# LabJunBMI/E3-invaraint-diffusion-model

Hardware: AMD Instinct MI355X
Metric: denoising-steps/sec (batched pocket graphs) (higher is better)
Workload: dtype f32 storage and accumulation, f16x3 products (fp32 grade); 1 GPU; structure_model sampling step, 256 x 256-residue pockets per GPU, 12+12 layers x 768, T=1000 schedule, encoder recomputed every step (as the reference); pockets_per_gpu=256, seq_len=256, parallelism=pocket-sharded x1, no collective

## Files before the change

e3-invaraint-diffusion-model_amd/csrc/attn_relkey_coop.hip:

```cpp
#include <type_traits>

#include "e3d_common.h"

namespace {

typedef __bf16 bf16x8 __attribute__((ext_vector_type(8)));
typedef __bf16 bf16x4 __attribute__((ext_vector_type(4)));
typedef _Float16 f16x8 __attribute__((ext_vector_type(8)));
typedef _Float16 f16x4 __attribute__((ext_vector_type(4)));
template <typename E> struct AV;
template <> struct AV<__bf16> { typedef bf16x8 x8; typedef bf16x4 x4; };
template <> struct AV<_Float16> { typedef f16x8 x8; typedef f16x4 x4; };
template <typename X> struct Elem;
template <> struct Elem<bf16x8> { typedef __bf16 type; };
template <> struct Elem<bf16x4> { typedef __bf16 type; };
template <> struct Elem<f16x8> { typedef _Float16 type; };
template <> struct Elem<f16x4> { typedef _Float16 type; };
__device__ __forceinline__ f32x16 mma16(const bf16x8 a, const bf16x8 b, const f32x16 c) {
    return __builtin_amdgcn_mfma_f32_32x32x16_bf16(a, b, c, 0, 0, 0);
}
__device__ __forceinline__ f32x16 mma16(const f16x8 a, const f16x8 b, const f32x16 c) {
    return __builtin_amdgcn_mfma_f32_32x32x16_f16(a, b, c, 0, 0, 0);
}

constexpr int D = 64;
constexpr int RING_LD = 34;
constexpr int RING_F = 64 * RING_LD;
constexpr int OUT_LD = 68;
constexpr int K_ROW_B = 144;
constexpr int V_ROW_B = 192;
constexpr int K_PLANE_B = 32 * K_ROW_B, V_PLANE_B = 32 * V_ROW_B;
constexpr float LOG2E = 1.4426950408889634f, LN2 = 0.6931471805599453f;
constexpr float Q_SCALE = 0.125f * LOG2E;
constexpr float MASK_BIAS = -10000.0f * LOG2E;
float g_rescale_tau = 8.0f;
constexpr int KV_BUF_B = 2 * K_PLANE_B + 2 * V_PLANE_B + 128;

template <typename X4>
__device__ __forceinline__ void split4x2(const f32x4 v, X4& hi, X4& lo) {
    typedef typename Elem<X4>::type E;
#pragma unroll
    for (int j = 0; j < 4; ++j) {
        const E p = (E)v[j];
        hi[j] = p;
        lo[j] = (E)(v[j] - (float)p);
    }
}

template <typename X8>
__device__ __forceinline__ void split8x2(const float (&x)[8], X8& hi, X8& lo) {
    typedef typename Elem<X8>::type E;
#pragma unroll
    for (int j = 0; j < 8; ++j) {
        const E p = (E)x[j];
        hi[j] = p;
        lo[j] = (E)(x[j] - (float)p);
    }
}

__device__ __forceinline__ void split4x2(const f32x4 v, f16x4& hi, f16x4& lo) {
    e3d_f16x2 h0, l0, h1, l1;
    e3d_split2_f16(v[0], v[1], h0, l0);
    e3d_split2_f16(v[2], v[3], h1, l1);
    hi = f16x4{h0[0], h0[1], h1[0], h1[1]};
    lo = f16x4{l0[0], l0[1], l1[0], l1[1]};
}
__device__ __forceinline__ void split8x2(const float (&x)[8], f16x8& hi, f16x8& lo) {
#pragma unroll
    for (int j = 0; j < 8; j += 2) {
        e3d_f16x2 h, l;
        e3d_split2_f16(x[j], x[j + 1], h, l);
        hi[j] = h[0]; hi[j + 1] = h[1];
        lo[j] = l[0]; lo[j + 1] = l[1];
    }
}

template <typename X8>
__device__ __forceinline__ f32x16 mfma3(const X8 (&a)[2], const X8 (&b)[2], f32x16 acc) {
    acc = mma16(a[0], b[1], acc);
    acc = mma16(a[1], b[0], acc);
    acc = mma16(a[0], b[0], acc);
    return acc;
}

typedef short short4v __attribute__((ext_vector_type(4)));
typedef short short8v __attribute__((ext_vector_type(8)));
template <typename X8>
__device__ __forceinline__ X8 tr_read8(const unsigned char* lo4, const unsigned char* hi4) {
    typedef __attribute__((address_space(3))) short4v* lds_p;
    const short4v a = __builtin_amdgcn_ds_read_tr16_b64_v4i16((lds_p)(lo4));
    const short4v b = __builtin_amdgcn_ds_read_tr16_b64_v4i16((lds_p)(hi4));
    const short8v c = __builtin_shufflevector(a, b, 0, 1, 2, 3, 4, 5, 6, 7);
    return __builtin_bit_cast(X8, c);
}

template <typename E>
__global__ __launch_bounds__(256) void e_fragments_kernel(const float* __restrict__ e, typename AV<E>::x8* __restrict__ frag,
                                                          int P, int J0, int n_items, float* __restrict__ e_absmax) {
    const int i = blockIdx.x * 256 + threadIdx.x;
    if (i >= n_items) return;
    const int lane = i & 63, kb = (i >> 6) & 3, plane = (i >> 8) & 1, j = i >> 9;
    const int row = min(max(P + 32 * (j - J0) + (lane & 31), 0), 2 * P - 2);
    const float* src = e + row * D + 16 * kb + 8 * (lane >> 5);
    typename AV<E>::x8 out;
    unsigned amax = 0;
#pragma unroll
    for (int t = 0; t < 8; ++t) {
        const float v = src[t];
        const E hi = (E)v;
        out[t] = plane ? (E)(v - (float)hi) : hi;
        e3d_absmax_accum(amax, v);
    }
    frag[i] = out;
    if (e_absmax && plane == 0) e3d_absmax_commit(amax, e_absmax, lane);
}

#ifdef E3D_ATTN_STAMPS
__device__ long long e3d_attn_stamps[16][8];
#define ASTAMP(slot)                                                                                     \
    do {                                                                                                 \
        if (blockIdx.x == 1000 && wid == 1 && lane == 0 && kt < 16) e3d_attn_stamps[kt][slot] = __builtin_readcyclecounter(); \
    } while (0)
#define KSTAMP(i)                                                                                        \
    do {                                                                                                 \
        if (blockIdx.x == 1000 && wid == 1 && lane == 0) e3d_attn_stamps[15][i] = __builtin_readcyclecounter(); \
    } while (0)
#else
#define ASTAMP(slot) do {} while (0)
#define KSTAMP(i) do {} while (0)
#endif

template <int W, bool RELKEY, typename E, bool DROP = false>
__global__ __launch_bounds__(W * 64, 2) void attn_coop_kernel(
    const float* __restrict__ q, int64_t q_bs, int64_t q_rs, const float* __restrict__ k, int64_t k_bs,
    int64_t k_rs, const float* __restrict__ v, int64_t v_bs, int64_t v_rs, const typename AV<E>::x8* __restrict__ e_frag,
    int P, const float* __restrict__ key_mask, float* __restrict__ out, float* __restrict__ lse, int nh, int Lq, int Lk,
    int groups_per_bh, int skip_padded_tiles, E3dBounds bnd, float rescale_tau, E3dDrop drop_in) {
    const E3dDrop drop = e3d_drop_resolve(drop_in);
    typedef typename AV<E>::x8 bf16x8;
    typedef typename AV<E>::x4 bf16x4;
    extern __shared__ __attribute__((aligned(16))) unsigned char smem_raw[];
    constexpr int NT = W * 64, NI = 512 / NT;
    const int tid = threadIdx.x, lane = tid & 63, wid = tid >> 6;
    const int qi = lane & 31, half = lane >> 5;
    const int blk = xcd_remap(blockIdx.x, gridDim.x);
    const int grp = blk % groups_per_bh, bh = blk / groups_per_bh, h = bh % nh, b = bh / nh;
    const int q0 = (grp * W + wid) * 32;
    float* ring = reinterpret_cast<float*>(smem_raw + 2 * KV_BUF_B) + wid * RING_F;
    KSTAMP(0);

    const float* kb_ = k + b * k_bs + h * D;
    const float* vb_ = v + b * v_bs + h * D;
    const float* mb = key_mask ? key_mask + (int64_t)b * Lk : nullptr;
    f32x4 qraw[8];
    {
        const float* qrow = q + b * q_bs + (int64_t)min(q0 + qi, Lq - 1) * q_rs + h * D + 8 * half;
#pragma unroll
        for (int kb = 0; kb < 4; ++kb) {
            qraw[2 * kb] = *reinterpret_cast<const f32x4*>(qrow + 16 * kb);
            qraw[2 * kb + 1] = *reinterpret_cast<const f32x4*>(qrow + 16 * kb + 4);
        }
    }
    const bool scan_mask = mb && skip_padded_tiles && e3d_mask_skip_is_exact(bnd);
    float mv[4];
    {
        const float* mp = mb ? mb : kb_;
#pragma unroll
        for (int c = 0; c < 4; ++c) mv[c] = mp[min(64 * c + lane, Lk - 1)];
    }

    bf16x8 qf[4][2];
    int k_tiles = (Lk + 31) >> 5;

    constexpr bool DEEP = NI <= 2;
    constexpr int NSET = DEEP ? 2 : 1;
    f32x4 sk[NSET][NI], sv[NSET][NI];
    float smask[NSET];
    int voff_k[NI], voff_v[NI];
#pragma unroll
    for (int i = 0; i < NI; ++i) {
        const int f = tid + NT * i;
        voff_k[i] = ((f >> 4) * (int)k_rs + 4 * (f & 15)) * 4;
        voff_v[i] = ((f >> 4) * (int)v_rs + 4 * (f & 15)) * 4;
    }
    const int voff_m = (tid & 31) * 4;
    auto tile_rsrc = [&](const float* base, int64_t rs, int r0, int tail_floats) {
        const int rows = Lk - r0;
        return __builtin_amdgcn_make_buffer_rsrc(const_cast<float*>(base + (int64_t)r0 * rs), 0,
                                                 (int)(((int64_t)(rows - 1) * rs + tail_floats) * 4), 0x00020000);
    };
    auto stage_load = [&](auto set_tag, int r0) {
        constexpr int SET = decltype(set_tag)::value;
        const auto rk = tile_rsrc(kb_, k_rs, r0, D), rv = tile_rsrc(vb_, v_rs, r0, D);
#pragma unroll
        for (int i = 0; i < NI; ++i) {
            sk[SET][i] = __builtin_bit_cast(f32x4, __builtin_amdgcn_raw_buffer_load_b128(rk, voff_k[i], 0, 0));
            sv[SET][i] = __builtin_bit_cast(f32x4, __builtin_amdgcn_raw_buffer_load_b128(rv, voff_v[i], 0, 0));
        }
        const auto rm = tile_rsrc(mb ? mb : kb_, 1, r0, 1);
        const float mval = __builtin_bit_cast(float, __builtin_amdgcn_raw_buffer_load_b32(rm, voff_m, 0, 0));
        smask[SET] = mb ? mval : 1.0f;
    };
    auto stage_store = [&](auto set_tag, int r0, unsigned char* buf) {
        constexpr int SET = decltype(set_tag)::value;
#pragma unroll
        for (int i = 0; i < NI; ++i) {
            const int f = tid + NT * i, row = f >> 4, c4 = f & 15;
            bf16x4 hi, lo;
            split4x2(sk[SET][i], hi, lo);
            *reinterpret_cast<bf16x4*>(buf + row * K_ROW_B + 8 * c4) = hi;
            *reinterpret_cast<bf16x4*>(buf + K_PLANE_B + row * K_ROW_B + 8 * c4) = lo;
            split4x2(sv[SET][i], hi, lo);
            *reinterpret_cast<bf16x4*>(buf + 2 * K_PLANE_B + row * V_ROW_B + 8 * c4) = hi;
            *reinterpret_cast<bf16x4*>(buf + 2 * K_PLANE_B + V_PLANE_B + row * V_ROW_B + 8 * c4) = lo;
        }
        if (tid < 32)
            reinterpret_cast<float*>(buf + 2 * K_PLANE_B + 2 * V_PLANE_B)[tid] =
                r0 + tid < Lk ? (1.0f - smask[SET]) * MASK_BIAS : -INFINITY;
    };
    using Set0 = std::integral_constant<int, 0>;
    using Set1 = std::integral_constant<int, DEEP ? 1 : 0>;

    bf16x8 ef[4][2];
    const int J0 = (Lk + 31) >> 5, qt = q0 >> 5;
    const auto e_rsrc = __builtin_amdgcn_make_buffer_rsrc(const_cast<bf16x8*>(e_frag ? e_frag : reinterpret_cast<const bf16x8*>(k)), 0,
                                                          2 * ((Lk + 31) >> 5) * 512 * 16, 0x00020000);
    const int voff_e = lane * 16;
    auto e_load = [&](int j) {
        const int so = __builtin_amdgcn_readfirstlane(j * 8192);
#pragma unroll
        for (int kb = 0; kb < 4; ++kb) {
            ef[kb][0] = __builtin_bit_cast(bf16x8, __builtin_amdgcn_raw_buffer_load_b128(e_rsrc, voff_e + kb * 1024, so, 0));
            ef[kb][1] = __builtin_bit_cast(bf16x8, __builtin_amdgcn_raw_buffer_load_b128(e_rsrc, voff_e + kb * 1024, so + 4096, 0));
        }
    };
    auto dot_q_acc = [&](const bf16x8 (&x)[4][2], f32x16 acc) {
#pragma unroll
        for (int kb = 0; kb < 4; ++kb) acc = mfma3(x[kb], qf[kb], acc);
        return acc;
    };
    auto dot_q = [&](const bf16x8 (&x)[4][2]) {
        f32x16 acc;
#pragma unroll
        for (int r = 0; r < 16; ++r) acc[r] = 0.f;
        return dot_q_acc(x, acc);
    };

    stage_load(Set0{}, 0);
    if (RELKEY) e_load(qt + J0);

    if (scan_mask) {
        int last = -1;
#pragma unroll
        for (int c = 0; c < 4; ++c) {
            const bool valid = 64 * c + lane < Lk && mv[c] != 0.f;
            const unsigned long long bits = __ballot(valid);
            if (bits) last = 64 * c + 63 - __builtin_clzll(bits);
        }
        for (int base = 256; base < Lk; base += 64) {
            const int key = base + lane;
            const bool valid = key < Lk && mb[key] != 0.f;
            const unsigned long long bits = __ballot(valid);
            if (bits) last = base + 63 - __builtin_clzll(bits);
        }
        if (last >= 0) k_tiles = (last >> 5) + 1;
    }
#pragma unroll
    for (int kb = 0; kb < 4; ++kb) {
        const f32x4 lo4 = qraw[2 * kb], hi4 = qraw[2 * kb + 1];
        float x[8] = {lo4[0] * Q_SCALE, lo4[1] * Q_SCALE, lo4[2] * Q_SCALE, lo4[3] * Q_SCALE,
                      hi4[0] * Q_SCALE, hi4[1] * Q_SCALE, hi4[2] * Q_SCALE, hi4[3] * Q_SCALE};
#pragma unroll
        for (int j = 0; j < 8; ++j) asm volatile("" : "+v"(x[j]));
        split8x2(x, qf[kb][0], qf[kb][1]);
    }
    if (RELKEY) {
        f32x16 t = dot_q(ef);
        e_load(qt - 1 + J0);
#pragma unroll
        for (int r = 0; r < 16; ++r) ring[(32 + mfma32_row(r, half)) * RING_LD + qi] = t[r];
        t = dot_q(ef);
        e_load(qt - (k_tiles > 1 ? 1 : 0) - 1 + J0);
#pragma unroll
        for (int r = 0; r < 16; ++r) ring[mfma32_row(r, half) * RING_LD + qi] = t[r];
    }
    stage_store(Set0{}, 0, smem_raw);
    if (DEEP) stage_load(Set1{}, (k_tiles > 1 ? 1 : 0) * 32);
    __syncthreads();
    KSTAMP(1);

    f32x16 o0, o1;
#pragma unroll
    for (int r = 0; r < 16; ++r) { o0[r] = 0.f; o1[r] = 0.f; }
    float m_run = 0.f, l_run = 0.f;
    float* const ring_w = ring + 4 * half * RING_LD + qi;
    const float* const ring_e = ring + (qi + 31 - 4 * half - 27) * RING_LD + qi;
    int rd_odd[16];
    if (RELKEY) {
#pragma unroll
        for (int r = 0; r < 16; ++r) rd_odd[r] = (((qi - mfma32_row(r, half) + 31) ^ 32) * RING_LD + qi);
    }

    auto tile = [&](auto par_tag, int kt) {
        constexpr int PAR = decltype(par_tag)::value;
        const unsigned char* buf = smem_raw + PAR * KV_BUF_B;
        const bool more = kt + 1 < k_tiles;
        const int kt_next = more ? kt + 1 : kt;
        ASTAMP(0);
        ASTAMP(1);

        const float* kbias = reinterpret_cast<const float*>(buf + 2 * K_PLANE_B + 2 * V_PLANE_B);
        f32x16 s;
#pragma unroll
        for (int g = 0; g < 4; ++g) {
            const f32x4 bv = *reinterpret_cast<const f32x4*>(kbias + 8 * g + 4 * half);
#pragma unroll
            for (int j = 0; j < 4; ++j) s[4 * g + j] = bv[j] - m_run;
        }
        if (RELKEY) {
#pragma unroll
            for (int r = 0; r < 16; ++r)
                s[r] += PAR ? ring[rd_odd[r]] : ring_e[(27 - ((r & 3) + 8 * (r >> 2))) * RING_LD];
        }
        {
            bf16x8 kf[4][2];
            const unsigned char* kr = buf + qi * K_ROW_B + 16 * half;
#pragma unroll
            for (int kb = 0; kb < 4; ++kb) {
                kf[kb][0] = *reinterpret_cast<const bf16x8*>(kr + 32 * kb);
                kf[kb][1] = *reinterpret_cast<const bf16x8*>(kr + K_PLANE_B + 32 * kb);
            }
            s = dot_q_acc(kf, s);
        }
        ASTAMP(2);
        const int kt_ld = DEEP ? (kt + 2 < k_tiles ? kt + 2 : k_tiles - 1) : kt_next;
        if (PAR == 0) stage_load(Set0{}, kt_ld * 32);
        else stage_load(Set1{}, kt_ld * 32);
        ASTAMP(3);

        float tmax = -INFINITY;
#pragma unroll
        for (int r = 0; r < 16; ++r) tmax = fmaxf(tmax, s[r]);
        tmax = fmaxf(tmax, __shfl_xor(tmax, 32, 64));
        const bool grow = kt == 0 || tmax > rescale_tau;
        if (__builtin_amdgcn_ballot_w64(grow) != 0ull) {
            const float delta = grow ? tmax : 0.f;
            const float alpha = kt == 0 ? 0.f : __builtin_amdgcn_exp2f(-delta);
            m_run += delta;
            l_run *= alpha;
#pragma unroll
            for (int r = 0; r < 16; ++r) { o0[r] *= alpha; o1[r] *= alpha; s[r] -= delta; }
        }
        float psum = 0.f;
#pragma unroll
        for (int r = 0; r < 16; ++r) {
            s[r] = __builtin_amdgcn_exp2f(s[r]);
            psum += s[r];
        }
        l_run += psum;
        if (DROP) {
#pragma unroll
            for (int g = 0; g < 4; ++g) {
                float m[4];
                e3d_drop_mult4(drop, e3d_attn_drop_idx4(bh, Lq, Lk, min(q0 + qi, Lq - 1), kt * 32 + 8 * g + 4 * half), m);
#pragma unroll
                for (int j = 0; j < 4; ++j) s[4 * g + j] *= m[j];
            }
        }
        ASTAMP(4);

        const unsigned char* vr = buf + 2 * K_PLANE_B + (4 * half + ((lane >> 2) & 3)) * V_ROW_B +
                                  2 * (16 * ((lane >> 4) & 1) + 4 * (lane & 3));
#pragma unroll
        for (int st = 0; st < 2; ++st) {
            float pv[8];
#pragma unroll
            for (int j = 0; j < 8; ++j) pv[j] = s[8 * st + j];
            bf16x8 pb[2], a0[2], a1[2];
            split8x2(pv, pb[0], pb[1]);
            const unsigned char* v0 = vr + 16 * st * V_ROW_B;
#pragma unroll
            for (int pl = 0; pl < 2; ++pl) {
                a0[pl] = tr_read8<bf16x8>(v0 + pl * V_PLANE_B, v0 + pl * V_PLANE_B + 8 * V_ROW_B);
                a1[pl] = tr_read8<bf16x8>(v0 + pl * V_PLANE_B + 64, v0 + pl * V_PLANE_B + 8 * V_ROW_B + 64);
            }
            o0 = mfma3(a0, pb, o0);
            o1 = mfma3(a1, pb, o1);
        }

        ASTAMP(5);
        if (more) {
            if (DEEP == (PAR == 0)) stage_store(Set1{}, kt_next * 32, smem_raw + (PAR ^ 1) * KV_BUF_B);
            else stage_store(Set0{}, kt_next * 32, smem_raw + (PAR ^ 1) * KV_BUF_B);
        }
        ASTAMP(6);
        if (RELKEY && more) {
            const f32x16 t = dot_q(ef);
            e_load(qt - (kt + 2 < k_tiles ? kt + 2 : k_tiles - 1) - 1 + J0);
#pragma unroll
            for (int r = 0; r < 16; ++r) ring_w[(32 * (PAR ^ 1) + (r & 3) + 8 * (r >> 2)) * RING_LD] = t[r];
        }
        __syncthreads();
        ASTAMP(7);
    };
    for (int kt = 0; kt < k_tiles; kt += 2) {
        tile(std::integral_constant<int, 0>{}, kt);
        if (kt + 1 < k_tiles) tile(std::integral_constant<int, 1>{}, kt + 1);
    }

    KSTAMP(2);
    const float l_tot = l_run + __shfl_xor(l_run, 32, 64);
    const float inv = 1.0f / l_tot;
    __builtin_amdgcn_wave_barrier();
#pragma unroll
    for (int g = 0; g < 4; ++g) {
        f32x4 a, c;
#pragma unroll
        for (int j = 0; j < 4; ++j) { a[j] = o0[4 * g + j] * inv; c[j] = o1[4 * g + j] * inv; }
        *reinterpret_cast<f32x4*>(ring + qi * OUT_LD + 8 * g + 4 * half) = a;
        *reinterpret_cast<f32x4*>(ring + qi * OUT_LD + 32 + 8 * g + 4 * half) = c;
    }
    __builtin_amdgcn_fence(__ATOMIC_RELEASE, "wavefront");
    __builtin_amdgcn_wave_barrier();
    __builtin_amdgcn_fence(__ATOMIC_ACQUIRE, "wavefront");
    float* obase = out + ((int64_t)b * Lq + q0) * (nh * D) + h * D;
#pragma unroll
    for (int i = 0; i < 8; ++i) {
        const int row = 4 * i + (lane >> 4);
        if (q0 + row < Lq)
            *reinterpret_cast<f32x4*>(obase + (int64_t)row * (nh * D) + 4 * (lane & 15)) =
                *reinterpret_cast<const f32x4*>(ring + row * OUT_LD + 4 * (lane & 15));
    }
    if (lse && half == 0 && q0 + qi < Lq) lse[((int64_t)b * nh + h) * Lq + q0 + qi] = m_run * LN2 + logf(l_tot);
    KSTAMP(3);
#ifdef E3D_ATTN_STAMPS
    asm volatile("s_waitcnt vmcnt(0)" ::: "memory");
    KSTAMP(4);
#endif
}

template <int W, bool RELKEY, typename E>
int launch_w(const float* q, int64_t q_bs, int64_t q_rs, const float* k, int64_t k_bs, int64_t k_rs, const float* v,
             int64_t v_bs, int64_t v_rs, const void* e_frag, int P, const float* key_mask,
             float* out, float* lse, int B, int nh, int Lq, int Lk, int q_tiles, int skip, E3dBounds bnd, E3dDrop drop,
             bool dropping, hipStream_t s) {
    const size_t lds = 2 * KV_BUF_B + (size_t)W * RING_F * sizeof(float);
    const int groups = q_tiles / W;
    if constexpr (std::is_same<E, __bf16>::value) {
        if (dropping) {
            static std::atomic<uint64_t> lds_ok_d{0};
            e3d_allow_lds(lds_ok_d, attn_coop_kernel<W, RELKEY, E, true>, lds);
            hipLaunchKernelGGL((attn_coop_kernel<W, RELKEY, E, true>), dim3(B * nh * groups), dim3(W * 64), lds, s, q, q_bs, q_rs,
                               k, k_bs, k_rs, v, v_bs, v_rs, reinterpret_cast<const typename AV<E>::x8*>(e_frag), P, key_mask,
                               out, lse, nh, Lq, Lk, groups, skip, bnd, g_rescale_tau, drop);
            return e3d_launch_status("e3d_relkey_attn_fwd_split (cooperative, dropout)");
        }
    }
    static std::atomic<uint64_t> lds_ok{0};
    e3d_allow_lds(lds_ok, attn_coop_kernel<W, RELKEY, E>, lds);
    hipLaunchKernelGGL((attn_coop_kernel<W, RELKEY, E>), dim3(B * nh * groups), dim3(W * 64), lds, s, q, q_bs, q_rs, k, k_bs,
                       k_rs, v, v_bs, v_rs, reinterpret_cast<const typename AV<E>::x8*>(e_frag), P, key_mask, out, lse, nh, Lq, Lk, groups, skip, bnd, g_rescale_tau, drop);
    return e3d_launch_status("e3d_relkey_attn_fwd_split (cooperative)");
}

template <bool RELKEY, typename E>
int launch_any(int W, const float* q, int64_t q_bs, int64_t q_rs, const float* k, int64_t k_bs, int64_t k_rs,
               const float* v, int64_t v_bs, int64_t v_rs, const void* e_frag, int P,
               const float* key_mask, float* out, float* lse, int B, int nh, int Lq, int Lk, int q_tiles, int skip,
               E3dBounds bnd, E3dDrop drop, bool dropping, hipStream_t s) {
#define E3D_COOP_CASE(w)                                                                                          \
    case w:                                                                                                       \
        return launch_w<w, RELKEY, E>(q, q_bs, q_rs, k, k_bs, k_rs, v, v_bs, v_rs, e_frag, P, key_mask, out, lse, B, nh, \
                                   Lq, Lk, q_tiles, skip, bnd, drop, dropping, s)
    switch (W) {
        E3D_COOP_CASE(8);
        E3D_COOP_CASE(4);
    }
#undef E3D_COOP_CASE
    return -1;
}

}

template <typename E>
static int coop_launch_t(const float* q, int64_t q_bs, int64_t q_rs, const float* k, int64_t k_bs, int64_t k_rs,
                         const float* v, int64_t v_bs, int64_t v_rs, const float* dist_emb, int P,
                         const float* key_mask, float* out, float* lse, int B, int nh, int Lq, int Lk, int skip,
                         E3dBounds bnd, void* e_scratch, int e_ready, E3dDrop drop, bool dropping, hipStream_t s) {
    const int q_tiles = (Lq + 31) / 32;
    static int w_pref = 0;
    if (!w_pref) {
        const char* e = getenv("E3D_ATTN_W");
        w_pref = e ? atoi(e) : 4;
    }
    const int W = (w_pref == 8 && q_tiles % 8 == 0) ? 8 : 4;
    if (!dist_emb)
        return launch_any<false, E>(W, q, q_bs, q_rs, k, k_bs, k_rs, v, v_bs, v_rs, nullptr, P, key_mask, out, lse, B, nh,
                                    Lq, Lk, q_tiles, skip, bnd, drop, dropping, s);
    if (!e_scratch) {
        e3d_set_error("attn_coop: rel-key attention needs the caller's scratch for the distance-table planes");
        return -1;
    }
    const int J0 = (Lk + 31) / 32, n_items = 2 * J0 * 512;
    if (!e_ready)
        hipLaunchKernelGGL(e_fragments_kernel<E>, dim3((n_items + 255) / 256), dim3(256), 0, s, dist_emb,
                           reinterpret_cast<typename AV<E>::x8*>(e_scratch), P, J0, n_items, (float*)nullptr);
    return launch_any<true, E>(W, q, q_bs, q_rs, k, k_bs, k_rs, v, v_bs, v_rs, e_scratch, P, key_mask, out, lse, B, nh, Lq,
                               Lk, q_tiles, skip, bnd, drop, dropping, s);
}

int e3d_attn_coop_launch(const float* q, int64_t q_bs, int64_t q_rs, const float* k, int64_t k_bs, int64_t k_rs,
                         const float* v, int64_t v_bs, int64_t v_rs, const float* dist_emb, int P,
                         const float* key_mask, float* out, float* lse, int B, int nh, int Lq, int Lk, int skip,
                         E3dBounds bnd, void* e_scratch, int e_ready, int f16, E3dDrop drop, bool dropping, hipStream_t s) {
    if (f16)
        return coop_launch_t<_Float16>(q, q_bs, q_rs, k, k_bs, k_rs, v, v_bs, v_rs, dist_emb, P, key_mask, out, lse, B, nh, Lq,
                                       Lk, skip, bnd, e_scratch, e_ready, drop, dropping, s);
    return coop_launch_t<__bf16>(q, q_bs, q_rs, k, k_bs, k_rs, v, v_bs, v_rs, dist_emb, P, key_mask, out, lse, B, nh, Lq, Lk,
                                 skip, bnd, e_scratch, e_ready, drop, dropping, s);
}

extern "C" float e3d_attn_rescale_tau(float tau) {
    const float prev = g_rescale_tau;
    if (tau >= 0.f) g_rescale_tau = tau;
    return prev;
}

#ifdef E3D_ATTN_STAMPS
extern "C" int e3d_debug_read_attn_stamps(long long* host_out) {
    return (int)hipMemcpyFromSymbol(host_out, HIP_SYMBOL(e3d_attn_stamps), sizeof(long long) * 16 * 8);
}
#endif

int e3d_attn_fill_planes(const float* dist_emb, int P, int Lk, void* scratch, int f16, float* e_absmax, hipStream_t s) {
    const int J0 = (Lk + 31) / 32, n_items = 2 * J0 * 512;
    if (f16)
        hipLaunchKernelGGL(e_fragments_kernel<_Float16>, dim3((n_items + 255) / 256), dim3(256), 0, s, dist_emb,
                           reinterpret_cast<f16x8*>(scratch), P, J0, n_items, e_absmax);
    else
        hipLaunchKernelGGL(e_fragments_kernel<__bf16>, dim3((n_items + 255) / 256), dim3(256), 0, s, dist_emb,
                           reinterpret_cast<bf16x8*>(scratch), P, J0, n_items, e_absmax);
    return e3d_launch_status("e3d_relkey_attn_fwd_split (distance-table planes)");
}

extern "C" int64_t e3d_attn_scratch_bytes(int Lk) { return (int64_t)2 * ((Lk + 31) / 32) * 512 * 16; }
```

e3-invaraint-diffusion-model_amd/csrc/attn_relkey_split.hip:

```cpp
#include "attn_split_frag.h"

namespace {

template <int NS, bool RELKEY, bool DROP, typename E>
__global__ __launch_bounds__(256, 2) void attn_fwd_split_kernel(
    const float* __restrict__ q, int64_t q_bs, int64_t q_rs, const float* __restrict__ k, int64_t k_bs,
    int64_t k_rs, const float* __restrict__ v, int64_t v_bs, int64_t v_rs, const float* __restrict__ dist_emb,
    int P, const float* __restrict__ key_mask, float* __restrict__ out, float* __restrict__ lse, int nh, int Lq,
    int Lk, int q_tiles, int n_units, int skip_padded_tiles, E3dBounds bnd, E3dDrop drop_in) {
    const E3dDrop drop = e3d_drop_resolve(drop_in);
    typedef typename AV<E>::x8 bf16x8;
    extern __shared__ __attribute__((aligned(16))) float smem[];
    const int lane = threadIdx.x & 63, wid = threadIdx.x >> 6;
    const int qi = lane & 31, half = lane >> 5;
    const int unit = xcd_remap(blockIdx.x, gridDim.x) * (blockDim.x >> 6) + wid;
    if (unit >= n_units) return;
    const int qt = unit % q_tiles, bh = unit / q_tiles, h = bh % nh, b = bh / nh;
    float* ring = smem + wid * WAVE_LDS_F;
    float* stg = ring + RING_F;
    float* kbias = stg + STG_F;

    const int q0 = qt * 32;
    const int lq = min(q0 + qi, Lq - 1);
    bf16x8 qf[4][NS];
    load_row_split<NS>(qf, q + b * q_bs + (int64_t)lq * q_rs + h * D, half);

    const float* kb_ = k + b * k_bs + h * D;
    const float* vb = v + b * v_bs + h * D;
    const float* mb = key_mask ? key_mask + (int64_t)b * Lk : nullptr;

    f32x16 o0, o1;
#pragma unroll
    for (int r = 0; r < 16; ++r) { o0[r] = 0.f; o1[r] = 0.f; }
    float m_run = -INFINITY, l_run = 0.f;

    int rot = 0;
    if (RELKEY) {
        TileRegs ereg;
        tile_load(ereg, dist_emb, D, q0 + 1 + P - 1, 0, 2 * P - 2, lane);
        bf16x8 ef[4][NS];
        tile_to_frags<NS>(ef, ereg, stg, lane);
        const f32x16 t = dot_tile<NS>(ef, qf);
#pragma unroll
        for (int r = 0; r < 16; ++r) ring[(32 + mfma32_row(r, half)) * RING_LD + qi] = t[r];
    }

    int k_tiles = (Lk + 31) >> 5;
    if (mb && skip_padded_tiles && e3d_mask_skip_is_exact(bnd)) {
        int last = -1;
        for (int base = 0; base < Lk; base += 64) {
            const int key = base + lane;
            const bool valid = key < Lk && mb[key] != 0.f;
            const unsigned long long bits = __ballot(valid);
            if (bits) last = base + 63 - __builtin_clzll(bits);
        }
        if (last >= 0) k_tiles = (last >> 5) + 1;
    }
    for (int kt = 0; kt < k_tiles; ++kt) {
        const int r0 = kt * 32;
        TileRegs kreg, ereg;
        VRegs vreg;
        tile_load(kreg, kb_, (int)k_rs, r0, 0, Lk - 1, lane);
        if (RELKEY) tile_load(ereg, dist_emb, D, q0 - r0 - 31 + P - 1, 0, 2 * P - 2, lane);
        {
            const int key = r0 + qi;
            float bias = -INFINITY;
            if (key < Lk) bias = mb ? (1.0f - mb[key]) * -10000.0f : 0.f;
            if (half == 0) kbias[qi] = bias;
        }
        f32x16 s;
        {
            bf16x8 kf[4][NS];
            tile_to_frags<NS>(kf, kreg, stg, lane);
            s = dot_tile<NS>(kf, qf);
        }
        if (RELKEY) {
            bf16x8 ef[4][NS];
            tile_to_frags<NS>(ef, ereg, stg, lane);
            const f32x16 t = dot_tile<NS>(ef, qf);
#pragma unroll
            for (int r = 0; r < 16; ++r) ring[((mfma32_row(r, half) + rot) & 63) * RING_LD + qi] = t[r];
            __builtin_amdgcn_fence(__ATOMIC_RELEASE, "wavefront");
            __builtin_amdgcn_wave_barrier();
            __builtin_amdgcn_fence(__ATOMIC_ACQUIRE, "wavefront");
#pragma unroll
            for (int r = 0; r < 16; ++r) {
                const int x = qi - mfma32_row(r, half) + 31;
                s[r] += ring[((x + rot) & 63) * RING_LD + qi];
            }
            __builtin_amdgcn_wave_barrier();
            rot ^= 32;
        }

        v_load(vreg, vb, (int)v_rs, r0, Lk, qi, half);
        float tmax = -INFINITY;
#pragma unroll
        for (int g = 0; g < 4; ++g) {
            const f32x4 bv = *reinterpret_cast<const f32x4*>(kbias + 8 * g + 4 * half);
#pragma unroll
            for (int j = 0; j < 4; ++j) {
                s[4 * g + j] = s[4 * g + j] * 0.125f + bv[j];
                tmax = fmaxf(tmax, s[4 * g + j]);
            }
        }
        tmax = fmaxf(tmax, __shfl_xor(tmax, 32, 64));
        const float m_new = fmaxf(m_run, tmax);
        const float alpha = fast_exp(m_run - m_new);
        m_run = m_new;
        float psum = 0.f;
#pragma unroll
        for (int r = 0; r < 16; ++r) {
            s[r] = fast_exp(s[r] - m_new);
            psum += s[r];
        }
        l_run = l_run * alpha + psum;
#pragma unroll
        for (int r = 0; r < 16; ++r) { o0[r] *= alpha; o1[r] *= alpha; }
        if (DROP) {
#pragma unroll
            for (int g = 0; g < 4; ++g) {
                float m[4];
                e3d_drop_mult4(drop, e3d_attn_drop_idx4(bh, Lq, Lk, q0 + qi, r0 + 8 * g + 4 * half), m);
#pragma unroll
                for (int j = 0; j < 4; ++j) s[4 * g + j] *= m[j];
            }
        }

#pragma unroll
        for (int st = 0; st < 2; ++st) {
            float pv[8], v0[8], v1[8];
#pragma unroll
            for (int j = 0; j < 8; ++j) {
                pv[j] = s[8 * st + j];
                v0[j] = vreg.v[8 * st + j].x;
                v1[j] = vreg.v[8 * st + j].y;
            }
            bf16x8 pb[NS], a0[NS], a1[NS];
            split8<NS>(pv, pb);
            split8<NS>(v0, a0);
            split8<NS>(v1, a1);
            o0 = mfma_terms<NS>(a0, pb, o0);
            o1 = mfma_terms<NS>(a1, pb, o1);
        }
    }

    const float l_tot = l_run + __shfl_xor(l_run, 32, 64);
    const float inv = 1.0f / l_tot;
    if (q0 + qi < Lq) {
        float* orow = out + ((int64_t)b * Lq + q0 + qi) * (nh * D) + h * D;
#pragma unroll
        for (int g = 0; g < 4; ++g) {
            f32x4 lo, hi;
            lo[0] = o0[4 * g + 0] * inv; lo[1] = o1[4 * g + 0] * inv;
            lo[2] = o0[4 * g + 1] * inv; lo[3] = o1[4 * g + 1] * inv;
            hi[0] = o0[4 * g + 2] * inv; hi[1] = o1[4 * g + 2] * inv;
            hi[2] = o0[4 * g + 3] * inv; hi[3] = o1[4 * g + 3] * inv;
            *reinterpret_cast<f32x4*>(orow + 16 * g + 8 * half) = lo;
            *reinterpret_cast<f32x4*>(orow + 16 * g + 8 * half + 4) = hi;
        }
        if (lse && half == 0) lse[((int64_t)b * nh + h) * Lq + q0 + qi] = m_run + logf(l_tot);
    }
}

int g_skip_padded = 1;

template <int NS, bool DROP = false, typename E = __bf16>
int launch(const float* q, int64_t q_bs, int64_t q_rs, const float* k, int64_t k_bs, int64_t k_rs, const float* v,
           int64_t v_bs, int64_t v_rs, const float* dist_emb, int P, const float* key_mask, float* out, float* lse,
           int B, int nh, int Lq, int Lk, E3dBounds bnd, hipStream_t s, E3dDrop drop = E3dDrop{0, 0, 1.f}) {
    const int q_tiles = (Lq + 31) / 32;
    const int n_units = B * nh * q_tiles;
    const int wpb = 4;
    const int n_blocks = (n_units + wpb - 1) / wpb;
    const size_t lds = (size_t)wpb * WAVE_LDS_F * sizeof(float);
    if (dist_emb)
        hipLaunchKernelGGL((attn_fwd_split_kernel<NS, true, DROP, E>), dim3(n_blocks), dim3(64 * wpb), lds, s, q, q_bs, q_rs, k,
                           k_bs, k_rs, v, v_bs, v_rs, dist_emb, P, key_mask, out, lse, nh, Lq, Lk, q_tiles, n_units, g_skip_padded, bnd, drop);
    else
        hipLaunchKernelGGL((attn_fwd_split_kernel<NS, false, DROP, E>), dim3(n_blocks), dim3(64 * wpb), lds, s, q, q_bs, q_rs, k,
                           k_bs, k_rs, v, v_bs, v_rs, dist_emb, P, key_mask, out, lse, nh, Lq, Lk, q_tiles, n_units, g_skip_padded, bnd, drop);
    return e3d_launch_status("e3d_relkey_attn_fwd_split");
}

}

extern "C" int e3d_attn_skip_padded_tiles(int enable) {
    const int prev = g_skip_padded;
    g_skip_padded = enable ? 1 : 0;
    return prev;
}

extern "C" int e3d_relkey_attn_fwd_split_ex(const float* q, int64_t q_bs, int64_t q_rs, const float* k, int64_t k_bs,
                                            int64_t k_rs, const float* v, int64_t v_bs, int64_t v_rs,
                                            const float* dist_emb, int P, const float* key_mask, float* out,
                                            float* lse, int B, int nh, int Lq, int Lk, int terms, float drop_p,
                                            uint64_t drop_seed, void* e_scratch, int e_scratch_ready, const float* q_absmax,
                                            const float* k_absmax, float* e_absmax, void* stream) {
    const E3dBounds bnd{q_absmax, k_absmax, dist_emb ? e_absmax : nullptr};
    E3D_REQUIRE(!dist_emb || !q_absmax || e_absmax, "attn_split: rel-key attention with element bounds needs e_absmax too");
    E3D_REQUIRE(drop_p >= 0.f && drop_p < 1.f, "attn_split: drop_p=%g outside [0, 1)", (double)drop_p);
    E3D_REQUIRE(q && k && v && out, "attn_split: null pointer");
    E3D_REQUIRE(B > 0 && nh > 0 && Lq > 0 && Lk > 0, "attn_split: bad shape B=%d nh=%d Lq=%d Lk=%d", B, nh, Lq, Lk);
    E3D_REQUIRE(q_rs % 4 == 0 && k_rs % 4 == 0 && v_rs % 2 == 0 && q_bs % 4 == 0 && k_bs % 4 == 0 && v_bs % 2 == 0,
                "attn_split: strides must keep 16B (q,k) / 8B (v) alignment");
    E3D_REQUIRE(((uintptr_t)q % 16) == 0 && ((uintptr_t)k % 16) == 0 && ((uintptr_t)v % 16) == 0 &&
                    ((uintptr_t)out % 16) == 0, "attn_split: pointers must be 16B aligned");
    E3D_REQUIRE(terms == 3 || terms == 6 || terms == E3D_TERMS_F16X3, "attn_split: terms must be 3, 6 or 19 (got %d)", terms);
    const int f16 = terms == E3D_TERMS_F16X3;
    E3D_REQUIRE((int64_t)Lk * k_rs < (1ll << 30) && (int64_t)Lk * v_rs < (1ll << 30),
                "attn_split: one batch item's K/V slab must stay below 2^30 elements (32-bit lane offsets)");
    if (dist_emb) {
        E3D_REQUIRE(Lq == Lk && Lq <= P, "attn_split: relative_key needs Lq == Lk <= P (Lq=%d Lk=%d P=%d)", Lq, Lk, P);
        E3D_REQUIRE(((uintptr_t)dist_emb % 16) == 0, "attn_split: dist_emb must be 16B aligned");
    }
    E3D_REQUIRE((int64_t)B * nh * ((Lq + 31) / 32) < (1ll << 30), "attn_split: too many tiles");
    hipStream_t s = (hipStream_t)stream;
    if (dist_emb && e_scratch && !e_scratch_ready) {
        const int rc = e3d_attn_fill_planes(dist_emb, P, Lk, e_scratch, f16, e_absmax, s);
        if (rc) return rc;
        e_scratch_ready = 1;
    }
    static int coop = -1;
    if (coop < 0) {
        const char* e = getenv("E3D_ATTN_COOP");
        coop = e ? atoi(e) : 1;
    }
    const bool dropping = drop_p > 0.f;
    const E3dDrop d = e3d_drop_make(drop_p, drop_seed);
    const bool span_ok = (int64_t)Lk * (k_rs > v_rs ? k_rs : v_rs) * 4 < ((int64_t)1 << 31) && k_rs > 0 && v_rs > 0 &&
                         k_rs < ((int64_t)1 << 24) && v_rs < ((int64_t)1 << 24);
    if ((terms == 3 || (f16 && !dropping)) && coop && span_ok && v_rs % 4 == 0 && v_bs % 4 == 0 && ((Lq + 31) / 32) % 4 == 0 &&
        (!dist_emb || e_scratch))
        return e3d_attn_coop_launch(q, q_bs, q_rs, k, k_bs, k_rs, v, v_bs, v_rs, dist_emb, P, key_mask, out, lse, B, nh,
                                    Lq, Lk, g_skip_padded, bnd, e_scratch, e_scratch_ready, f16, d, dropping, s);
    if (dropping) {
        if (terms == 3)
            return launch<2, true>(q, q_bs, q_rs, k, k_bs, k_rs, v, v_bs, v_rs, dist_emb, P, key_mask, out, lse, B, nh, Lq, Lk, bnd, s, d);
        return launch<3, true>(q, q_bs, q_rs, k, k_bs, k_rs, v, v_bs, v_rs, dist_emb, P, key_mask, out, lse, B, nh, Lq, Lk, bnd, s, d);
    }
    if (f16)
        return launch<2, false, _Float16>(q, q_bs, q_rs, k, k_bs, k_rs, v, v_bs, v_rs, dist_emb, P, key_mask, out, lse, B, nh,
                                          Lq, Lk, bnd, s);
    if (terms == 3)
        return launch<2>(q, q_bs, q_rs, k, k_bs, k_rs, v, v_bs, v_rs, dist_emb, P, key_mask, out, lse, B, nh, Lq, Lk, bnd, s);
    return launch<3>(q, q_bs, q_rs, k, k_bs, k_rs, v, v_bs, v_rs, dist_emb, P, key_mask, out, lse, B, nh, Lq, Lk, bnd, s);
}

extern "C" int e3d_relkey_attn_fwd_split(const float* q, int64_t q_bs, int64_t q_rs, const float* k, int64_t k_bs,
                                         int64_t k_rs, const float* v, int64_t v_bs, int64_t v_rs,
                                         const float* dist_emb, int P, const float* key_mask, float* out, float* lse,
                                         int B, int nh, int Lq, int Lk, int terms, void* stream) {
    return e3d_relkey_attn_fwd_split_ex(q, q_bs, q_rs, k, k_bs, k_rs, v, v_bs, v_rs, dist_emb, P, key_mask, out, lse, B,
                                        nh, Lq, Lk, terms, 0.f, 0, nullptr, 0, nullptr, nullptr, nullptr, stream);
}

extern "C" int e3d_relkey_attn_fwd_split_drop(const float* q, int64_t q_bs, int64_t q_rs, const float* k, int64_t k_bs,
                                              int64_t k_rs, const float* v, int64_t v_bs, int64_t v_rs,
                                              const float* dist_emb, int P, const float* key_mask, float* out,
                                              float* lse, int B, int nh, int Lq, int Lk, int terms, float drop_p,
                                              uint64_t drop_seed, void* stream) {
    return e3d_relkey_attn_fwd_split_ex(q, q_bs, q_rs, k, k_bs, k_rs, v, v_bs, v_rs, dist_emb, P, key_mask, out, lse, B,
                                        nh, Lq, Lk, terms, drop_p, drop_seed, nullptr, 0, nullptr, nullptr, nullptr, stream);
}
```

e3-invaraint-diffusion-model_amd/csrc/e3d_common.h:

```cpp
#pragma once
#include <hip/hip_runtime.h>
#include <stdint.h>
#include <stdio.h>
#include <math.h>
#include <atomic>

#include "../../include/e3d_hip.h"

typedef float f32x4 __attribute__((ext_vector_type(4)));
typedef float f32x16 __attribute__((ext_vector_type(16)));

void e3d_set_error(const char* fmt, ...);

struct E3dBounds { const float* q; const float* k; const float* e; };


#define E3D_REQUIRE(cond, ...)       \
    do {                             \
        if (!(cond)) {               \
            e3d_set_error(__VA_ARGS__); \
            return -1;               \
        }                            \
    } while (0)

static inline int e3d_current_device() {
    int d = 0;
    (void)hipGetDevice(&d);
    return d;
}
template <typename F>
static inline void e3d_once_per_device(std::atomic<uint64_t>& mask, F&& f) {
    const int d = e3d_current_device();
    const uint64_t bit = 1ull << (d & 63);
    if (!(mask.load(std::memory_order_acquire) & bit)) {
        f(d);
        mask.fetch_or(bit, std::memory_order_release);
    }
}
static inline int e3d_cu_count() {
    static std::atomic<int> n_cu[64];
    const int d = e3d_current_device() & 63;
    int n = n_cu[d].load(std::memory_order_relaxed);
    if (!n) {
        if (hipDeviceGetAttribute(&n, hipDeviceAttributeMultiprocessorCount, d) != hipSuccess || n <= 0) n = 256;
        n -= n % 8;
        if (n <= 0) n = 8;
        n_cu[d].store(n, std::memory_order_relaxed);
    }
    return n;
}
template <typename K>
static inline void e3d_allow_lds(std::atomic<uint64_t>& mask, K kernel, size_t lds_bytes) {
    e3d_once_per_device(mask, [&](int) {
        (void)hipFuncSetAttribute(reinterpret_cast<const void*>(kernel), hipFuncAttributeMaxDynamicSharedMemorySize,
                                  (int)lds_bytes);
    });
}

static __global__ void e3d_zero_kernel(float* __restrict__ p, size_t n) {
    for (size_t i = (size_t)blockIdx.x * blockDim.x + threadIdx.x; i < n; i += (size_t)gridDim.x * blockDim.x) p[i] = 0.f;
}
static inline hipError_t e3d_zero_async(float* p, size_t n_floats, hipStream_t s) {
    if (n_floats == 0) return hipSuccess;
    const size_t blocks = (n_floats + 1023) / 1024;
    hipLaunchKernelGGL(e3d_zero_kernel, dim3((unsigned)(blocks < 2048 ? blocks : 2048)), dim3(256), 0, s, p, n_floats);
    return hipGetLastError();
}
static __global__ void e3d_zero2d_kernel(float* __restrict__ p, size_t ld, size_t rows, size_t cols) {
    const size_t n = rows * cols;
    for (size_t i = (size_t)blockIdx.x * blockDim.x + threadIdx.x; i < n; i += (size_t)gridDim.x * blockDim.x)
        p[(i / cols) * ld + i % cols] = 0.f;
}

static inline int e3d_launch_status(const char* what) {
    hipError_t e = hipGetLastError();
    if (e != hipSuccess) {
        e3d_set_error("%s: %s", what, hipGetErrorString(e));
        return (int)e;
    }
    return 0;
}

__device__ __forceinline__ int mfma32_row(int reg, int half) {
    return (reg & 3) + 8 * (reg >> 2) + 4 * half;
}

__device__ __forceinline__ float gelu_erf(float x) {
    const float ax = fabsf(x), z = ax * 0.70710678118654752440f;
    const float t = __builtin_amdgcn_rcpf(fmaf(0.3275911f, z, 1.0f));
    float p = fmaf(1.061405429f, t, -1.453152027f);
    p = fmaf(p, t, 1.421413741f);
    p = fmaf(p, t, -0.284496736f);
    p = fmaf(p, t, 0.254829592f);
    const float erfc_z = p * t * __builtin_amdgcn_exp2f(-1.4426950408889634f * z * z);
    return fmaxf(x, 0.f) - 0.5f * ax * erfc_z;
}

__device__ __forceinline__ float silu(float x) { return x / (1.0f + expf(-x)); }

typedef _Float16 e3d_f16x2 __attribute__((ext_vector_type(2)));
__device__ __forceinline__ void e3d_split2_f16(float x0, float x1, e3d_f16x2& hi, e3d_f16x2& lo) {
    e3d_f16x2 p;
    p[0] = (_Float16)x0;
    p[1] = (_Float16)x1;
    float r0, r1;
    asm("v_fma_mix_f32 %0, %1, -1.0, %2 op_sel_hi:[1,0,0]" : "=v"(r0) : "v"(p), "v"(x0));
    asm("v_fma_mix_f32 %0, %1, -1.0, %2 op_sel:[1,0,0] op_sel_hi:[1,0,0]" : "=v"(r1) : "v"(p), "v"(x1));
    hi = p;
    lo[0] = (_Float16)r0;
    lo[1] = (_Float16)r1;
}


__device__ __forceinline__ float wave_sum(float v) {
#pragma unroll
    for (int o = 32; o > 0; o >>= 1) v += __shfl_xor(v, o, 64);
    return v;
}

__device__ __forceinline__ void e3d_absmax_accum(unsigned& m, float v) {
    const unsigned b = __float_as_uint(v) & 0x7fffffffu;
    m = m > b ? m : b;
}
__device__ __forceinline__ void e3d_absmax_commit(unsigned m, float* target, int lane) {
#pragma unroll
    for (int o = 32; o > 0; o >>= 1) {
        const unsigned t = (unsigned)__shfl_xor((int)m, o, 64);
        m = m > t ? m : t;
    }
    if (lane == 0) {
        unsigned* t = reinterpret_cast<unsigned*>(target);
        if (m > __hip_atomic_load(t, __ATOMIC_RELAXED, __HIP_MEMORY_SCOPE_AGENT)) atomicMax(t, m);
    }
}
__device__ __forceinline__ bool e3d_mask_skip_is_exact(const E3dBounds b) {
    if (!b.q || !b.k) return false;
    const float qa = *b.q, ka = *b.k, ea = b.e ? *b.e : 0.f;
    return 16.0f * qa * (ka + ea) < 9890.0f;
}

struct E3dDrop {
    uint64_t seed;
    uint32_t thr;
    float scale;
    const uint64_t* epoch;
};
const uint64_t* e3d_dropout_epoch_ptr();
static inline E3dDrop e3d_drop_make(float p, uint64_t seed) {
    E3dDrop d;
    long t = lrintf(p * 65536.0f);
    t = t < 0 ? 0 : (t > 65535 ? 65535 : t);
    d.seed = seed;
    d.epoch = e3d_dropout_epoch_ptr();
    d.thr = (uint32_t)t;
    d.scale = 65536.0f / (float)(65536 - t);
    return d;
}
__device__ __forceinline__ E3dDrop e3d_drop_resolve(E3dDrop d) {
    if (d.epoch) d.seed += *d.epoch * 0xD1342543DE82EF95ull;
    d.epoch = nullptr;
    return d;
}
__device__ __forceinline__ void e3d_drop_mult4(const E3dDrop d, uint64_t idx4, float (&m)[4]) {
    uint64_t z = idx4 + d.seed * 0x9E3779B97F4A7C15ull + 0x9E3779B97F4A7C15ull;
    z = (z ^ (z >> 30)) * 0xBF58476D1CE4E5B9ull;
    z = (z ^ (z >> 27)) * 0x94D049BB133111EBull;
    z ^= z >> 31;
#pragma unroll
    for (int j = 0; j < 4; ++j) m[j] = ((uint32_t)(z >> (16 * j)) & 0xFFFFu) >= d.thr ? d.scale : 0.f;
}
__device__ __forceinline__ uint64_t e3d_attn_drop_idx4(int bh, int Lq, int Lk, int q, int key0) {
    return ((uint64_t)bh * Lq + q) * (uint64_t)((Lk + 3) >> 2) + (uint64_t)(key0 >> 2);
}

int e3d_attn_fill_planes(const float* dist_emb, int P, int Lk, void* scratch, int f16, float* e_absmax, hipStream_t s);

int e3d_attn_coop_launch(const float* q, int64_t q_bs, int64_t q_rs, const float* k, int64_t k_bs, int64_t k_rs,
                         const float* v, int64_t v_bs, int64_t v_rs, const float* dist_emb, int P,
                         const float* key_mask, float* out, float* lse, int B, int nh, int Lq, int Lk, int skip,
                         E3dBounds bnd, void* e_scratch, int e_ready, int f16, E3dDrop drop, bool dropping, hipStream_t s);

int e3d_attn_bwd_split_launch(const float* q, int64_t q_bs, int64_t q_rs, const float* k, int64_t k_bs, int64_t k_rs,
                              const float* v, int64_t v_bs, int64_t v_rs, const float* dist_emb, int P,
                              const float* key_mask, const float* out, const float* lse, const float* dout, float* dq,
                              int64_t dq_bs, int64_t dq_rs, float* dk, int64_t dk_bs, int64_t dk_rs, float* dv,
                              int64_t dv_bs, int64_t dv_rs, float* Pm, float* dSm, float* part, int B, int nh, int Lq,
                              int Lk, E3dDrop drop, bool dropping, hipStream_t s);

int64_t e3d_attn_bwd_coop_scratch_bytes(int Lk);
int64_t e3d_attn_bwd_coop_de_floats(int Lq, int Lk);
bool e3d_attn_bwd_coop_supported(int Lq, int Lk, bool dropping);
int e3d_attn_bwd_coop_launch(const float* q, int64_t q_bs, int64_t q_rs, const float* k, int64_t k_bs, int64_t k_rs,
                             const float* v, int64_t v_bs, int64_t v_rs, const float* dist_emb, int P,
                             const float* key_mask, const float* out, const float* lse, const float* dout, float* dq,
                             int64_t dq_bs, int64_t dq_rs, float* dk, int64_t dk_bs, int64_t dk_rs, float* dv,
                             int64_t dv_bs, int64_t dv_rs, float* d_dist_emb, void* e_scratch, float* part, int B, int nh,
                             int Lq, int Lk, E3dDrop drop, bool dropping, hipStream_t s);

__device__ __forceinline__ int xcd_remap(int id, int n) {
    const int q = n >> 3, r = n & 7, xcd = id & 7, slot = id >> 3;
    return (xcd < r ? xcd * (q + 1) : r * (q + 1) + (xcd - r) * q) + slot;
}
```

Baseline: 3813 pocket-steps/s.

## Precompute key-mask bias once per block in LDS and hoist buffer descriptors

New measurement: 3825 pocket-steps/s, median of 6. About the same (+0.3%).

```diff
diff --git a/e3-invaraint-diffusion-model_amd/csrc/attn_relkey_coop.hip b/e3-invaraint-diffusion-model_amd/csrc/attn_relkey_coop.hip
--- a/e3-invaraint-diffusion-model_amd/csrc/attn_relkey_coop.hip
+++ b/e3-invaraint-diffusion-model_amd/csrc/attn_relkey_coop.hip
@@ -34,7 +34,10 @@
 constexpr float Q_SCALE = 0.125f * LOG2E;
 constexpr float MASK_BIAS = -10000.0f * LOG2E;
 float g_rescale_tau = 8.0f;
-constexpr int KV_BUF_B = 2 * K_PLANE_B + 2 * V_PLANE_B + 128;
+constexpr int KV_BUF_B = 2 * K_PLANE_B + 2 * V_PLANE_B;
+constexpr size_t coop_lds_bytes(int W, int Lk) {
+    return 2 * (size_t)KV_BUF_B + (size_t)W * RING_F * sizeof(float) + (size_t)((Lk + 31) / 32) * 32 * sizeof(float);
+}
 
 template <typename X4>
 __device__ __forceinline__ void split4x2(const f32x4 v, X4& hi, X4& lo) {
@@ -147,6 +150,7 @@
     const int grp = blk % groups_per_bh, bh = blk / groups_per_bh, h = bh % nh, b = bh / nh;
     const int q0 = (grp * W + wid) * 32;
     float* ring = reinterpret_cast<float*>(smem_raw + 2 * KV_BUF_B) + wid * RING_F;
+    float* const kbias_all = reinterpret_cast<float*>(smem_raw + 2 * KV_BUF_B) + W * RING_F;
     KSTAMP(0);
 
     const float* kb_ = k + b * k_bs + h * D;
@@ -175,7 +179,6 @@
     constexpr bool DEEP = NI <= 2;
     constexpr int NSET = DEEP ? 2 : 1;
     f32x4 sk[NSET][NI], sv[NSET][NI];
-    float smask[NSET];
     int voff_k[NI], voff_v[NI];
 #pragma unroll
     for (int i = 0; i < NI; ++i) {
@@ -183,25 +186,19 @@
         voff_k[i] = ((f >> 4) * (int)k_rs + 4 * (f & 15)) * 4;
         voff_v[i] = ((f >> 4) * (int)v_rs + 4 * (f & 15)) * 4;
     }
-    const int voff_m = (tid & 31) * 4;
-    auto tile_rsrc = [&](const float* base, int64_t rs, int r0, int tail_floats) {
-        const int rows = Lk - r0;
-        return __builtin_amdgcn_make_buffer_rsrc(const_cast<float*>(base + (int64_t)r0 * rs), 0,
-                                                 (int)(((int64_t)(rows - 1) * rs + tail_floats) * 4), 0x00020000);
+    const auto rk = __builtin_amdgcn_make_buffer_rsrc(const_cast<float*>(kb_), 0, (int)(((int64_t)(Lk - 1) * k_rs + D) * 4), 0x00020000);
+    const auto rv = __builtin_amdgcn_make_buffer_rsrc(const_cast<float*>(vb_), 0, (int)(((int64_t)(Lk - 1) * v_rs + D) * 4), 0x00020000);
+    const int k_tile_b = (int)k_rs * 128, v_tile_b = (int)v_rs * 128;
+    auto stage_load = [&](auto set_tag, int kt) {
+        constexpr int SET = decltype(set_tag)::value;
+        const int ko = kt * k_tile_b, vo = kt * v_tile_b;
+#pragma unroll
+        for (int i = 0; i < NI; ++i) {
+            sk[SET][i] = __builtin_bit_cast(f32x4, __builtin_amdgcn_raw_buffer_load_b128(rk, voff_k[i] + ko, 0, 0));
+            sv[SET][i] = __builtin_bit_cast(f32x4, __builtin_amdgcn_raw_buffer_load_b128(rv, voff_v[i] + vo, 0, 0));
+        }
     };
-    auto stage_load = [&](auto set_tag, int r0) {
-        constexpr int SET = decltype(set_tag)::value;
-        const auto rk = tile_rsrc(kb_, k_rs, r0, D), rv = tile_rsrc(vb_, v_rs, r0, D);
-#pragma unroll
-        for (int i = 0; i < NI; ++i) {
-            sk[SET][i] = __builtin_bit_cast(f32x4, __builtin_amdgcn_raw_buffer_load_b128(rk, voff_k[i], 0, 0));
-            sv[SET][i] = __builtin_bit_cast(f32x4, __builtin_amdgcn_raw_buffer_load_b128(rv, voff_v[i], 0, 0));
-        }
-        const auto rm = tile_rsrc(mb ? mb : kb_, 1, r0, 1);
-        const float mval = __builtin_bit_cast(float, __builtin_amdgcn_raw_buffer_load_b32(rm, voff_m, 0, 0));
-        smask[SET] = mb ? mval : 1.0f;
-    };
-    auto stage_store = [&](auto set_tag, int r0, unsigned char* buf) {
+    auto stage_store = [&](auto set_tag, unsigned char* buf) {
         constexpr int SET = decltype(set_tag)::value;
 #pragma unroll
         for (int i = 0; i < NI; ++i) {
@@ -214,9 +211,6 @@
             *reinterpret_cast<bf16x4*>(buf + 2 * K_PLANE_B + row * V_ROW_B + 8 * c4) = hi;
             *reinterpret_cast<bf16x4*>(buf + 2 * K_PLANE_B + V_PLANE_B + row * V_ROW_B + 8 * c4) = lo;
         }
-        if (tid < 32)
-            reinterpret_cast<float*>(buf + 2 * K_PLANE_B + 2 * V_PLANE_B)[tid] =
-                r0 + tid < Lk ? (1.0f - smask[SET]) * MASK_BIAS : -INFINITY;
     };
     using Set0 = std::integral_constant<int, 0>;
     using Set1 = std::integral_constant<int, DEEP ? 1 : 0>;
@@ -249,6 +243,15 @@
     stage_load(Set0{}, 0);
     if (RELKEY) e_load(qt + J0);
 
+    if (wid == 0) {
+#pragma unroll
+        for (int c = 0; c < 4; ++c) {
+            const int key = 64 * c + lane;
+            if (key < 32 * J0) kbias_all[key] = key < Lk ? (1.0f - (mb ? mv[c] : 1.0f)) * MASK_BIAS : -INFINITY;
+        }
+    }
+    for (int key = 256 + tid; key < 32 * J0; key += NT)
+        kbias_all[key] = key < Lk ? (1.0f - (mb ? mb[key] : 1.0f)) * MASK_BIAS : -INFINITY;
     if (scan_mask) {
         int last = -1;
 #pragma unroll
@@ -274,18 +277,19 @@
         for (int j = 0; j < 8; ++j) asm volatile("" : "+v"(x[j]));
         split8x2(x, qf[kb][0], qf[kb][1]);
     }
+    float* const ring_w = ring + (4 - 4 * half) * RING_LD + qi;
     if (RELKEY) {
         f32x16 t = dot_q(ef);
         e_load(qt - 1 + J0);
 #pragma unroll
-        for (int r = 0; r < 16; ++r) ring[(32 + mfma32_row(r, half)) * RING_LD + qi] = t[r];
+        for (int r = 0; r < 16; ++r) ring_w[(27 - ((r & 3) + 8 * (r >> 2))) * RING_LD] = t[r];
         t = dot_q(ef);
         e_load(qt - (k_tiles > 1 ? 1 : 0) - 1 + J0);
 #pragma unroll
-        for (int r = 0; r < 16; ++r) ring[mfma32_row(r, half) * RING_LD + qi] = t[r];
-    }
-    stage_store(Set0{}, 0, smem_raw);
-    if (DEEP) stage_load(Set1{}, (k_tiles > 1 ? 1 : 0) * 32);
+        for (int r = 0; r < 16; ++r) ring_w[(59 - ((r & 3) + 8 * (r >> 2))) * RING_LD] = t[r];
+    }
+    stage_store(Set0{}, smem_raw);
+    if (DEEP) stage_load(Set1{}, k_tiles > 1 ? 1 : 0);
     __syncthreads();
     KSTAMP(1);
 
@@ -293,12 +297,11 @@
 #pragma unroll
     for (int r = 0; r < 16; ++r) { o0[r] = 0.f; o1[r] = 0.f; }
     float m_run = 0.f, l_run = 0.f;
-    float* const ring_w = ring + 4 * half * RING_LD + qi;
-    const float* const ring_e = ring + (qi + 31 - 4 * half - 27) * RING_LD + qi;
+    const float* const ring_e = ring + (32 - qi + 4 * half) * RING_LD + qi;
     int rd_odd[16];
     if (RELKEY) {
 #pragma unroll
-        for (int r = 0; r < 16; ++r) rd_odd[r] = (((qi - mfma32_row(r, half) + 31) ^ 32) * RING_LD + qi);
+        for (int r = 0; r < 16; ++r) rd_odd[r] = ((63 - ((qi - mfma32_row(r, half) + 31) ^ 32)) * RING_LD + qi);
     }
 
     auto tile = [&](auto par_tag, int kt) {
@@ -309,7 +312,7 @@
         ASTAMP(0);
         ASTAMP(1);
 
-        const float* kbias = reinterpret_cast<const float*>(buf + 2 * K_PLANE_B + 2 * V_PLANE_B);
+        const float* kbias = kbias_all + 32 * kt;
         f32x16 s;
 #pragma unroll
         for (int g = 0; g < 4; ++g) {
@@ -320,7 +323,7 @@
         if (RELKEY) {
 #pragma unroll
             for (int r = 0; r < 16; ++r)
-                s[r] += PAR ? ring[rd_odd[r]] : ring_e[(27 - ((r & 3) + 8 * (r >> 2))) * RING_LD];
+                s[r] += PAR ? ring[rd_odd[r]] : ring_e[((r & 3) + 8 * (r >> 2)) * RING_LD];
         }
         {
             bf16x8 kf[4][2];
@@ -334,8 +337,8 @@
         }
         ASTAMP(2);
         const int kt_ld = DEEP ? (kt + 2 < k_tiles ? kt + 2 : k_tiles - 1) : kt_next;
-        if (PAR == 0) stage_load(Set0{}, kt_ld * 32);
-        else stage_load(Set1{}, kt_ld * 32);
+        if (PAR == 0) stage_load(Set0{}, kt_ld);
+        else stage_load(Set1{}, kt_ld);
         ASTAMP(3);
 
         float tmax = -INFINITY;
@@ -390,15 +393,15 @@
 
         ASTAMP(5);
         if (more) {
-            if (DEEP == (PAR == 0)) stage_store(Set1{}, kt_next * 32, smem_raw + (PAR ^ 1) * KV_BUF_B);
-            else stage_store(Set0{}, kt_next * 32, smem_raw + (PAR ^ 1) * KV_BUF_B);
+            if (DEEP == (PAR == 0)) stage_store(Set1{}, smem_raw + (PAR ^ 1) * KV_BUF_B);
+            else stage_store(Set0{}, smem_raw + (PAR ^ 1) * KV_BUF_B);
         }
         ASTAMP(6);
         if (RELKEY && more) {
             const f32x16 t = dot_q(ef);
             e_load(qt - (kt + 2 < k_tiles ? kt + 2 : k_tiles - 1) - 1 + J0);
 #pragma unroll
-            for (int r = 0; r < 16; ++r) ring_w[(32 * (PAR ^ 1) + (r & 3) + 8 * (r >> 2)) * RING_LD] = t[r];
+            for (int r = 0; r < 16; ++r) ring_w[(59 - 32 * (PAR ^ 1) - ((r & 3) + 8 * (r >> 2))) * RING_LD] = t[r];
         }
         __syncthreads();
         ASTAMP(7);
@@ -444,12 +447,16 @@
              int64_t v_bs, int64_t v_rs, const void* e_frag, int P, const float* key_mask,
              float* out, float* lse, int B, int nh, int Lq, int Lk, int q_tiles, int skip, E3dBounds bnd, E3dDrop drop,
              bool dropping, hipStream_t s) {
-    const size_t lds = 2 * KV_BUF_B + (size_t)W * RING_F * sizeof(float);
+    const size_t lds = coop_lds_bytes(W, Lk), lds_max = coop_lds_bytes(W, E3D_ATTN_COOP_MAX_LK);
+    if (lds > lds_max) {
+        e3d_set_error("attn_coop: key length beyond E3D_ATTN_COOP_MAX_LK (the dispatcher sends such shapes to the per-wave kernel)");
+        return -1;
+    }
     const int groups = q_tiles / W;
     if constexpr (std::is_same<E, __bf16>::value) {
         if (dropping) {
             static std::atomic<uint64_t> lds_ok_d{0};
-            e3d_allow_lds(lds_ok_d, attn_coop_kernel<W, RELKEY, E, true>, lds);
+            e3d_allow_lds(lds_ok_d, attn_coop_kernel<W, RELKEY, E, true>, lds_max);
             hipLaunchKernelGGL((attn_coop_kernel<W, RELKEY, E, true>), dim3(B * nh * groups), dim3(W * 64), lds, s, q, q_bs, q_rs,
                                k, k_bs, k_rs, v, v_bs, v_rs, reinterpret_cast<const typename AV<E>::x8*>(e_frag), P, key_mask,
                                out, lse, nh, Lq, Lk, groups, skip, bnd, g_rescale_tau, drop);
@@ -457,7 +464,7 @@
         }
     }
     static std::atomic<uint64_t> lds_ok{0};
-    e3d_allow_lds(lds_ok, attn_coop_kernel<W, RELKEY, E>, lds);
+    e3d_allow_lds(lds_ok, attn_coop_kernel<W, RELKEY, E>, lds_max);
     hipLaunchKernelGGL((attn_coop_kernel<W, RELKEY, E>), dim3(B * nh * groups), dim3(W * 64), lds, s, q, q_bs, q_rs, k, k_bs,
                        k_rs, v, v_bs, v_rs, reinterpret_cast<const typename AV<E>::x8*>(e_frag), P, key_mask, out, lse, nh, Lq, Lk, groups, skip, bnd, g_rescale_tau, drop);
     return e3d_launch_status("e3d_relkey_attn_fwd_split (cooperative)");
diff --git a/e3-invaraint-diffusion-model_amd/csrc/attn_relkey_split.hip b/e3-invaraint-diffusion-model_amd/csrc/attn_relkey_split.hip
--- a/e3-invaraint-diffusion-model_amd/csrc/attn_relkey_split.hip
+++ b/e3-invaraint-diffusion-model_amd/csrc/attn_relkey_split.hip
@@ -229,7 +229,7 @@
     const E3dDrop d = e3d_drop_make(drop_p, drop_seed);
     const bool span_ok = (int64_t)Lk * (k_rs > v_rs ? k_rs : v_rs) * 4 < ((int64_t)1 << 31) && k_rs > 0 && v_rs > 0 &&
                          k_rs < ((int64_t)1 << 24) && v_rs < ((int64_t)1 << 24);
-    if ((terms == 3 || (f16 && !dropping)) && coop && span_ok && v_rs % 4 == 0 && v_bs % 4 == 0 && ((Lq + 31) / 32) % 4 == 0 &&
+    if ((terms == 3 || (f16 && !dropping)) && coop && span_ok && Lk <= E3D_ATTN_COOP_MAX_LK && v_rs % 4 == 0 && v_bs % 4 == 0 && ((Lq + 31) / 32) % 4 == 0 &&
         (!dist_emb || e_scratch))
         return e3d_attn_coop_launch(q, q_bs, q_rs, k, k_bs, k_rs, v, v_bs, v_rs, dist_emb, P, key_mask, out, lse, B, nh,
                                     Lq, Lk, g_skip_padded, bnd, e_scratch, e_scratch_ready, f16, d, dropping, s);
diff --git a/e3-invaraint-diffusion-model_amd/csrc/e3d_common.h b/e3-invaraint-diffusion-model_amd/csrc/e3d_common.h
--- a/e3-invaraint-diffusion-model_amd/csrc/e3d_common.h
+++ b/e3-invaraint-diffusion-model_amd/csrc/e3d_common.h
@@ -175,6 +175,7 @@
 
 int e3d_attn_fill_planes(const float* dist_emb, int P, int Lk, void* scratch, int f16, float* e_absmax, hipStream_t s);
 
+constexpr int E3D_ATTN_COOP_MAX_LK = 8192;
 int e3d_attn_coop_launch(const float* q, int64_t q_bs, int64_t q_rs, const float* k, int64_t k_bs, int64_t k_rs,
                          const float* v, int64_t v_bs, int64_t v_rs, const float* dist_emb, int P,
                          const float* key_mask, float* out, float* lse, int B, int nh, int Lq, int Lk, int skip,
```
